# zhukovanadezhda/collaborative-filtering

Hardware: AMD Instinct MI355X
Metric: ratings/sec per ALS iteration at k=64 (higher is better)
Workload: dtype f32 (storage, solve, accumulate); Gram products as 2-way fp16 split (error <= 2^-23) on fp16 MFMA; rows over the condition limit redone in f64 (solve_dtype=auto)

## Files before the change

### collaborative-filtering_amd/csrc/row_solve.hip

```cpp
#include <type_traits>
#include "als_device.hpp"
#include "als_hip.h"
#include "row_common.hpp"
#include "slot_fold.hpp"

namespace {

template <int KB>
struct RowAcc {
    f32x4 acc[KCfg<KB>::NACC];
    float rhs[KB];
    float cs[KB];
    float sumr;
    float sumr2;
    __device__ __forceinline__ void zero() {
#pragma unroll
        for (int a = 0; a < KCfg<KB>::NACC; ++a) acc[a] = f32x4{0.f, 0.f, 0.f, 0.f};
#pragma unroll
        for (int b = 0; b < KB; ++b) { rhs[b] = 0.f; cs[b] = 0.f; }
        sumr = 0.f; sumr2 = 0.f;
    }
};

template <int KB, bool FULL>
__device__ __forceinline__ void process_chunk(RowAcc<KB>& A, int off_l, float r_l, int nvalid,
                                              const float* __restrict__ Fc, int q) {
    constexpr int GS = KCfg<KB>::GS;
#pragma unroll
    for (int g0 = 0; g0 < 16; g0 += GS) {
        if (!FULL && 4 * g0 >= nvalid) break;
        float f[GS][KB];
        int off_t[GS];
        float r_t[GS];
#pragma unroll
        for (int s = 0; s < GS; ++s) {
            const int src = FULL ? 16 * q + g0 + s : 4 * (g0 + s) + q;
            off_t[s] = bperm_i(off_l, src);
            r_t[s] = bperm_f(r_l, src);
        }
#pragma unroll
        for (int s = 0; s < GS; ++s)
            if (FULL || 4 * (g0 + s) < nvalid) load_frow<KB>(Fc + (uint32_t)off_t[s], f[s]);
#pragma unroll
        for (int s = 0; s < GS; ++s) {
            if (FULL || 4 * (g0 + s) < nvalid) {
#pragma unroll
                for (int b = 0; b < KB; ++b) {
                    A.rhs[b] = fmaf(f[s][b], r_t[s], A.rhs[b]);
                    A.cs[b] += f[s][b];
                }
#pragma unroll
                for (int bi = 0; bi < KB; ++bi)
#pragma unroll
                    for (int bj = 0; bj <= bi; ++bj)
                        A.acc[blk_idx(bi, bj)] = __builtin_amdgcn_mfma_f32_16x16x4f32(
                            f[s][bi], f[s][bj], A.acc[blk_idx(bi, bj)], 0, 0, 0);
            }
        }
    }
}


template <int KB, bool FULL>
__device__ __forceinline__ void process_chunk_f16x2(RowAcc<KB>& A, int off_l, float r_l, int nvalid,
                                                    const float* __restrict__ Fc, int q, float S) {
#pragma unroll
    for (int g = 0; g < 2; ++g) {
        if (!FULL && 32 * g >= nvalid) break;
        int off_t[8];
        float r_t[8];
        float f[8][KB];
#pragma unroll
        for (int j = 0; j < 8; ++j) {
            const int src = FULL ? 16 * q + 8 * g + j : 32 * g + 8 * q + j;
            off_t[j] = bperm_i(off_l, src);
            r_t[j] = bperm_f(r_l, src);
        }
#pragma unroll
        for (int j = 0; j < 8; ++j) load_frow<KB>(Fc + (uint32_t)off_t[j], f[j]);
        i32x4 H[KB], L[KB];
#pragma unroll
        for (int b = 0; b < KB; ++b) {
#pragma unroll
            for (int j = 0; j < 8; j += 2) {
                const float x0 = f[j][b], x1 = f[j + 1][b];
                A.rhs[b] = fmaf(x0, r_t[j], A.rhs[b]);
                A.rhs[b] = fmaf(x1, r_t[j + 1], A.rhs[b]);
                A.cs[b] += x0 + x1;
                int hw, lw;
                split2(x0, x1, S, hw, lw);
                H[b][j >> 1] = hw; L[b][j >> 1] = lw;
            }
        }
#pragma unroll
        for (int bi = 0; bi < KB; ++bi)
#pragma unroll
            for (int bj = 0; bj <= bi; ++bj) {
                f32x4 acc = A.acc[blk_idx(bi, bj)];
                const h16x8 hi = __builtin_bit_cast(h16x8, H[bi]), hj = __builtin_bit_cast(h16x8, H[bj]);
                const h16x8 li = __builtin_bit_cast(h16x8, L[bi]), lj = __builtin_bit_cast(h16x8, L[bj]);
                acc = __builtin_amdgcn_mfma_f32_16x16x32_f16(li, hj, acc, 0, 0, 0);
                acc = __builtin_amdgcn_mfma_f32_16x16x32_f16(hi, lj, acc, 0, 0, 0);
                acc = __builtin_amdgcn_mfma_f32_16x16x32_f16(hi, hj, acc, 0, 0, 0);
                A.acc[blk_idx(bi, bj)] = acc;
            }
    }
}

template <int KB, bool FULL>
__device__ __forceinline__ void process_chunk_planes(RowAcc<KB>& A, f32x4 (&E)[KB], int off_l, int rp_l, int nvalid,
                                                     const uint32_t* __restrict__ Pc, int q, int sel_c, int ones_c) {
    static_assert(KB == 4 || KB == 8, "pre-split operands: k = 49 ... 64 and 113 ... 128");
    constexpr int NW = KB / 2;
    typedef uint32_t u32x4 __attribute__((ext_vector_type(4)));
#pragma unroll
    for (int g = 0; g < 2; ++g) {
        if (!FULL && 32 * g >= nvalid) break;
        int off_t[8], rp_t[8];
#pragma unroll
        for (int j = 0; j < 8; ++j) {
            const int src = FULL ? 16 * q + 8 * g + j : 32 * g + 8 * q + j;
            off_t[j] = bperm_i(off_l, src);
            rp_t[j] = bperm_i(rp_l, src);
        }
        uint32_t w[8][KB];
#pragma unroll
        for (int j = 0; j < 8; ++j)
#pragma unroll
            for (int v4 = 0; v4 < KB / 4; ++v4) {
                const u32x4 t = *reinterpret_cast<const u32x4*>(Pc + (uint32_t)off_t[j] + 4 * v4);
                w[j][4 * v4] = t[0]; w[j][4 * v4 + 1] = t[1]; w[j][4 * v4 + 2] = t[2]; w[j][4 * v4 + 3] = t[3];
            }
        i32x4 H[KB], L[KB], R;
#pragma unroll
        for (int d = 0; d < 4; ++d) {
            R[d] = (int)__builtin_amdgcn_perm((uint32_t)rp_t[2 * d + 1], (uint32_t)rp_t[2 * d], (uint32_t)sel_c) | ones_c;
#pragma unroll
            for (int b = 0; b < KB; ++b) {
                const uint32_t sel = (b & 1) ? 0x07060302u : 0x05040100u;
                H[b][d] = (int)__builtin_amdgcn_perm(w[2 * d + 1][b >> 1], w[2 * d][b >> 1], sel);
                L[b][d] = (int)__builtin_amdgcn_perm(w[2 * d + 1][NW + (b >> 1)], w[2 * d][NW + (b >> 1)], sel);
            }
        }
        const h16x8 rr = __builtin_bit_cast(h16x8, R);
#pragma unroll
        for (int bi = 0; bi < KB; ++bi) {
            const h16x8 hi = __builtin_bit_cast(h16x8, H[bi]), li = __builtin_bit_cast(h16x8, L[bi]);
            E[bi] = __builtin_amdgcn_mfma_f32_16x16x32_f16(rr, li, E[bi], 0, 0, 0);
            E[bi] = __builtin_amdgcn_mfma_f32_16x16x32_f16(rr, hi, E[bi], 0, 0, 0);
#pragma unroll
            for (int bj = 0; bj <= bi; ++bj) {
                f32x4 acc = A.acc[blk_idx(bi, bj)];
                const h16x8 hj = __builtin_bit_cast(h16x8, H[bj]), lj = __builtin_bit_cast(h16x8, L[bj]);
                acc = __builtin_amdgcn_mfma_f32_16x16x32_f16(li, hj, acc, 0, 0, 0);
                acc = __builtin_amdgcn_mfma_f32_16x16x32_f16(hi, lj, acc, 0, 0, 0);
                acc = __builtin_amdgcn_mfma_f32_16x16x32_f16(hi, hj, acc, 0, 0, 0);
                A.acc[blk_idx(bi, bj)] = acc;
            }
        }
    }
}

template <int KB>
__device__ __forceinline__ void fold_planes_rhs(RowAcc<KB>& A, f32x4 (&E)[KB], int q, float inv_s) {
#pragma unroll
    for (int b = 0; b < KB; ++b) {
        A.rhs[b] += (q == 0) ? (E[b][0] + E[b][2]) * inv_s : 0.f;
        A.cs[b] += (q == 0) ? E[b][1] * inv_s : 0.f;
        E[b] = f32x4{0.f, 0.f, 0.f, 0.f};
    }
}

constexpr int FLUSH_GROUPS = 16;

template <int KB>
__device__ __forceinline__ void flush_acc(RowAcc<KB>& A, float* __restrict__ Ls, int lane, bool first) {
    if (!first) {
#pragma unroll
        for (int a = 0; a < KCfg<KB>::NACC; ++a)
#pragma unroll
            for (int r = 0; r < 4; ++r) A.acc[a][r] += Ls[(a * 4 + r) * 64 + lane];
    }
#pragma unroll
    for (int a = 0; a < KCfg<KB>::NACC; ++a)
#pragma unroll
        for (int r = 0; r < 4; ++r) {
            Ls[(a * 4 + r) * 64 + lane] = A.acc[a][r];
            A.acc[a][r] = 0.f;
        }
}

template <int KB>
__device__ __forceinline__ void unflush_acc(RowAcc<KB>& A, const float* __restrict__ Ls, int lane) {
#pragma unroll
    for (int a = 0; a < KCfg<KB>::NACC; ++a)
#pragma unroll
        for (int r = 0; r < 4; ++r) A.acc[a][r] += Ls[(a * 4 + r) * 64 + lane];
}

template <int KB, int MODE>
__device__ __forceinline__ void gram_accumulate(RowAcc<KB>& A, const int32_t* __restrict__ idxp,
                                                const float* __restrict__ valp, int len,
                                                const float* __restrict__ F, int ld, int zero_row,
                                                const float* __restrict__ bias_other, float mu,
                                                float bself, int lane, float* __restrict__ Ls, float S,
                                                const uint32_t* __restrict__ planes = nullptr) {
    const int c = lane & 15, q = lane >> 4;
    const float* Fc = F + KB * c;
    int nflush = 0;
    f32x4 E[MODE == 2 ? KB : 1];
    const uint32_t* Pc = planes + KB * c;
    const int sel_c = (c == 0) ? 0x05040100 : (c == 2) ? 0x07060302 : 0x0c0c0c0c;
    const int ones_c = (c == 1) ? 0x3C003C00 : 0;
    const float inv_s = __int_as_float((254 - ((__float_as_int(S) >> 23) & 0xff)) << 23);
    if constexpr (MODE == 2) {
#pragma unroll
        for (int b = 0; b < KB; ++b) E[b] = f32x4{0.f, 0.f, 0.f, 0.f};
    }
    int idx1 = (lane < len) ? __builtin_nontemporal_load(idxp + lane) : zero_row;
    int idx2 = (64 + lane < len) ? __builtin_nontemporal_load(idxp + 64 + lane) : zero_row;
    float val1 = (lane < len) ? __builtin_nontemporal_load(valp + lane) : 0.f;
    float bo1 = (lane < len) ? bias_other[idx1] : 0.f;
    for (int base = 0; base < len; base += 64) {
        const int idx0 = idx1;
        const float val0 = val1, bo0 = bo1;
        idx1 = idx2;
        const int t2 = base + 128 + lane;
        idx2 = (t2 < len) ? __builtin_nontemporal_load(idxp + t2) : zero_row;
        const int t1 = base + 64 + lane;
        val1 = (t1 < len) ? __builtin_nontemporal_load(valp + t1) : 0.f;
        bo1 = (t1 < len) ? bias_other[idx1] : 0.f;
        const int nvalid = min(64, len - base);
        const bool ok = lane < nvalid;
        const float rb = val0 - mu - bo0;
        A.sumr += ok ? rb : 0.f;
        A.sumr2 = ok ? fmaf(rb, rb, A.sumr2) : A.sumr2;
        const float r0 = ok ? (rb - bself) : 0.f;
        const int off0 = idx0 * ld;
        if constexpr (MODE == 0) {
            if (nvalid == 64) process_chunk<KB, true>(A, off0, r0, 64, Fc, q);
            else              process_chunk<KB, false>(A, off0, r0, nvalid, Fc, q);
        } else {
            if constexpr (MODE == 2) {
                const _Float16 rh = (_Float16)r0;
                const _Float16 rl = (_Float16)(r0 - (float)rh);
                const int rp = (int)__builtin_bit_cast(unsigned short, rh) | ((int)__builtin_bit_cast(unsigned short, rl) << 16);
                if (nvalid == 64) process_chunk_planes<KB, true>(A, E, off0, rp, 64, Pc, q, sel_c, ones_c);
                else              process_chunk_planes<KB, false>(A, E, off0, rp, nvalid, Pc, q, sel_c, ones_c);
            } else {
                if (nvalid == 64) process_chunk_f16x2<KB, true>(A, off0, r0, 64, Fc, q, S);
                else              process_chunk_f16x2<KB, false>(A, off0, r0, nvalid, Fc, q, S);
            }
            if (((base >> 6) + 1) % (FLUSH_GROUPS / 2) == 0 && base + 64 < len) {
                mfma_results_settle();
                if constexpr (MODE == 2) fold_planes_rhs<KB>(A, E, q, inv_s);
                flush_acc<KB>(A, Ls, lane, nflush == 0);
                ++nflush;
            }
        }
    }
    if (MODE != 0) mfma_results_settle();
    if constexpr (MODE == 2) fold_planes_rhs<KB>(A, E, q, inv_s);
    if (MODE != 0 && nflush > 0) {
        unflush_acc<KB>(A, Ls, lane);
        wave_lds_sync();
    }
}

template <int KB>
__device__ __forceinline__ void store_partial(const RowAcc<KB>& A, float* __restrict__ ws, int lane) {
    int it = 0;
#pragma unroll
    for (int a = 0; a < KCfg<KB>::NACC; ++a)
#pragma unroll
        for (int r = 0; r < 4; ++r) ws[(it++) * 64 + lane] = A.acc[a][r];
#pragma unroll
    for (int b = 0; b < KB; ++b) ws[(it++) * 64 + lane] = A.rhs[b];
#pragma unroll
    for (int b = 0; b < KB; ++b) ws[(it++) * 64 + lane] = A.cs[b];
    ws[(it++) * 64 + lane] = A.sumr;
    ws[it * 64 + lane] = A.sumr2;
}

template <int KB>
__device__ __forceinline__ void add_partial(RowAcc<KB>& A, const float* __restrict__ ws, int lane) {
    int it = 0;
#pragma unroll
    for (int a = 0; a < KCfg<KB>::NACC; ++a)
#pragma unroll
        for (int r = 0; r < 4; ++r) A.acc[a][r] += ws[(it++) * 64 + lane];
#pragma unroll
    for (int b = 0; b < KB; ++b) A.rhs[b] += ws[(it++) * 64 + lane];
#pragma unroll
    for (int b = 0; b < KB; ++b) A.cs[b] += ws[(it++) * 64 + lane];
    A.sumr += ws[(it++) * 64 + lane];
    A.sumr2 += ws[it * 64 + lane];
}

template <int KB, int J, int T, bool SOLVE>
__device__ __forceinline__ void panel_pivot(float (&p)[KCfg<KB>::NR][16], Chol<KB>& S, int lane) {
    constexpr int NR = KCfg<KB>::NR;
    constexpr int PIV = 16 * J + T, RP = PIV >> 6, LP = PIV & 63;
    constexpr int DR = (16 * J) >> 6, DL = (16 * J) & 63;
    const float prep = bperm_f(p[DR][T], DL + (lane & 15));
    const float d = readlane_f(p[RP][T], LP);
    const float inv = __builtin_amdgcn_rsqf(d);
    float l[NR];
#pragma unroll
    for (int rr = 0; rr < NR; ++rr) { l[rr] = p[rr][T] * inv; p[rr][T] = l[rr]; }
    float lrep = -(prep * inv);
    asm("s_nop 1" : "+v"(lrep));
    float yt = 0.f;
    if constexpr (SOLVE) yt = readlane_f(S.b[RP], LP) * inv;
    panel_trailing<KB, T + 1>(p, l, lrep);
    if constexpr (SOLVE) {
#pragma unroll
        for (int rr = 0; rr < NR; ++rr) S.b[rr] = fmaf(-l[rr], yt, S.b[rr]);
        S.y[RP] = select_lanes<1ull << LP>(yt, S.y[RP]);
    }
}

template <int KB, int J, int T, bool SOLVE>
__device__ __forceinline__ void panel_pivots(float (&p)[KCfg<KB>::NR][16], Chol<KB>& S, int lane) {
    if constexpr (T < 16) {
        panel_pivot<KB, J, T, SOLVE>(p, S, lane);
        panel_pivots<KB, J, T + 1, SOLVE>(p, S, lane);
    }
}

template <int KB, int J, bool SOLVE>
__device__ __forceinline__ void chol_panel(RowAcc<KB>& A, Chol<KB>& S, float* __restrict__ Ls, int lane) {
    using C = KCfg<KB>;
    constexpr int KP = C::KP, NR = C::NR;
    constexpr int OFF = C::lcol_off(J);
    const int c = lane & 15, q = lane >> 4;
    {
        const int swzc = (((c >> 2) ^ q) << 2) + (c & 3);
#pragma unroll
        for (int I = J; I < KB; ++I)
#pragma unroll
            for (int r = 0; r < 4; ++r)
                Ls[OFF + (16 * (I - J) + 4 * q + r) * 16 + swzc] = A.acc[blk_idx(I, J)][r];
    }
    wave_lds_sync();
    float p[NR][16];
    const int si = (lane >> 2) & 3;
#pragma unroll
    for (int rr = 0; rr < NR; ++rr) {
        const int i = lane + 64 * rr;
        const int rowi = min(max(i, 16 * J), KP - 1) - 16 * J;
#pragma unroll
        for (int g = 0; g < 4; ++g) {
            const f32x4 v = *reinterpret_cast<const f32x4*>(Ls + OFF + rowi * 16 + ((g ^ si) << 2));
            p[rr][4 * g] = v.x; p[rr][4 * g + 1] = v.y; p[rr][4 * g + 2] = v.z; p[rr][4 * g + 3] = v.w;
        }
    }
    wave_lds_sync();
    panel_pivots<KB, J, 0, SOLVE>(p, S, lane);
#pragma unroll
    for (int rr = 0; rr < NR; ++rr) {
        const int i = lane + 64 * rr;
        if (i >= 16 * J && i < KP) {
#pragma unroll
            for (int g = 0; g < 4; ++g) {
                const f32x4 v = {p[rr][4 * g], p[rr][4 * g + 1], p[rr][4 * g + 2], p[rr][4 * g + 3]};
                *reinterpret_cast<f32x4*>(Ls + OFF + (i - 16 * J) * 16 + ((g ^ si) << 2)) = v;
            }
        }
    }
    wave_lds_sync();
    {
        constexpr int DR = (16 * J) >> 6, DL = (16 * J) & 63;
        const float dl = Ls[OFF + c * 16 + (c & 3)];
        S.di[DR] = select_lanes<0xFFFFull << DL>(__builtin_amdgcn_rcpf(dl), S.di[DR]);
    }
    if constexpr (J + 1 < KB) {
        f32x4 op[KB - J - 1];
        const int sg = ((q ^ ((c >> 2) & 3)) << 2);
#pragma unroll
        for (int I = J + 1; I < KB; ++I)
            op[I - J - 1] = *reinterpret_cast<const f32x4*>(Ls + OFF + (16 * (I - J) + c) * 16 + sg);
#pragma unroll
        for (int K = J + 1; K < KB; ++K) {
            const f32x4 nb = -op[K - J - 1];
#pragma unroll
            for (int I = K; I < KB; ++I)
#pragma unroll
                for (int e = 0; e < 4; ++e)
                    A.acc[blk_idx(I, K)] = __builtin_amdgcn_mfma_f32_16x16x4f32(
                        op[I - J - 1][e], nb[e], A.acc[blk_idx(I, K)], 0, 0, 0);
        }
    }
}

template <int KB, int J, bool SOLVE>
__device__ __forceinline__ void chol_panels(RowAcc<KB>& A, Chol<KB>& S, float* __restrict__ Ls, int lane) {
    if constexpr (J < KB) {
        chol_panel<KB, J, SOLVE>(A, S, Ls, lane);
        chol_panels<KB, J + 1, SOLVE>(A, S, Ls, lane);
    }
}

template <int KB>
__device__ __forceinline__ bool row_needs_f64(const Chol<KB>& S, const als_row_solve_params& P, int row, bool spd,
                                              float mean_eig, float short_row_bound, int lane) {
    float dmx = 0.f, dmn = 0.f;
#pragma unroll
    for (int rr = 0; rr < KCfg<KB>::NR; ++rr) {
        const bool in = lane + 64 * rr < KCfg<KB>::KP;
        const float d = in ? S.di[rr] : 0.f;
        dmx = fmaxf(dmx, d);
        dmn = fmaxf(dmn, in ? __builtin_amdgcn_rcpf(d) : 0.f);
    }
    dmx = wave_max_nonneg(fmaxf(dmx, 0.f));
    dmn = wave_max_nonneg(fmaxf(dmn, 0.f));
    const float r = dmx * dmn;
    const float kappa = spd ? fmaxf(fmaxf(r * r, mean_eig * dmx * dmx), short_row_bound) : __builtin_inff();
    if (P.cond_out && lane == 0) P.cond_out[row] = kappa;
    const bool redo = !(kappa <= P.cond_limit);
    if (redo && lane == 0) P.redo_rows[atomicAdd(P.redo_count, 1)] = row;
    return redo;
}

template <int KB>
__device__ __forceinline__ float gram_trace(const RowAcc<KB>& A, int lane) {
    const int c = lane & 15, q = lane >> 4;
    float t = 0.f;
#pragma unroll
    for (int J = 0; J < KB; ++J) {
        const f32x4 a = A.acc[blk_idx(J, J)];
        const float lo = (c & 1) ? a[1] : a[0], hi = (c & 1) ? a[3] : a[2];
        t += (c & 2) ? hi : lo;
    }
    return wave_sum((q == (c >> 2)) ? t : 0.f);
}

template <int KB>
__device__ __forceinline__ void finish_row(RowAcc<KB>& A, const als_row_solve_params& P, int row,
                                           float* __restrict__ Ls, int lane) {
    using C = KCfg<KB>;
    constexpr int KP = C::KP, NR = C::NR;
    const int c = lane & 15, q = lane >> 4;
    const int64_t r64 = row;

    if (P.gram_mode == ALS_GRAM_F16X2) {
        const float un = P.F_scale[1];
#pragma unroll
        for (int a = 0; a < C::NACC; ++a) A.acc[a] *= un;
    }

#pragma unroll
    for (int b = 0; b < KB; ++b) {
        A.rhs[b] += __shfl_xor(A.rhs[b], 16, 64); A.rhs[b] += __shfl_xor(A.rhs[b], 32, 64);
        A.cs[b] += __shfl_xor(A.cs[b], 16, 64);   A.cs[b] += __shfl_xor(A.cs[b], 32, 64);
    }
    const float sumr = wave_sum(A.sumr);
    const float sumr2 = wave_sum(A.sumr2);

    Chol<KB> S;
    float csrow[NR];
    int colrow[NR];
#pragma unroll
    for (int rr = 0; rr < NR; ++rr) {
        float bsel = 0.f, csel = 0.f;
#pragma unroll
        for (int e = 0; e < 4; ++e) {
            constexpr int dummy = 0; (void)dummy;
            const int b = (4 * rr + e < KB) ? 4 * rr + e : KB - 1;
            if (4 * rr + e < KB) {
                bsel = (q == e) ? A.rhs[b] : bsel;
                csel = (q == e) ? A.cs[b] : csel;
            }
        }
        S.b[rr] = bsel; S.di[rr] = 0.f; S.y[rr] = 0.f;
        csrow[rr] = csel;
        colrow[rr] = perm_to_col<KB>(min(lane + 64 * rr, KP - 1));
    }

    if (P.gram_out) {
        float* G = P.gram_out + r64 * KP * KP;
#pragma unroll
        for (int I = 0; I < KB; ++I)
#pragma unroll
            for (int K = 0; K <= I; ++K)
#pragma unroll
                for (int r = 0; r < 4; ++r)
                    G[(16 * I + 4 * q + r) * KP + 16 * K + c] = A.acc[blk_idx(I, K)][r];
    }
#pragma unroll
    for (int rr = 0; rr < NR; ++rr) {
        const int i = lane + 64 * rr;
        if (i < KP) {
            if (P.rhs_out) P.rhs_out[r64 * KP + i] = S.b[rr];
            if (P.colsum_out) P.colsum_out[r64 * KP + i] = csrow[rr];
        }
    }
    if (P.sumr_out && lane == 0) P.sumr_out[row] = sumr;
    if (P.sumr2_out && lane == 0) P.sumr2_out[row] = sumr2;

    const float lam = (P.lambda_row ? P.lambda_row[row] : P.lambda_scalar) + ALS_EPS
                    + (P.diag_extra ? P.diag_extra[row] : 0.f);
    float mean_eig = 0.f, short_row_bound = 0.f;
    if (P.cond_limit > 0.f) {
        const int64_t nrat = P.indptr[row + 1] - P.indptr[row];
        mean_eig = gram_trace<KB>(A, lane) / fmaxf((float)min((int64_t)P.k, nrat), 1.f) + lam;
        short_row_bound = (nrat < 4 * (int64_t)P.k) ? mean_eig / lam : 0.f;
    }
#pragma unroll
    for (int J = 0; J < KB; ++J) {
        const float dv = (perm_to_col<KB>(16 * J + c) < P.k) ? lam : 1.0f;
#pragma unroll
        for (int r = 0; r < 4; ++r) A.acc[blk_idx(J, J)][r] += (4 * q + r == c) ? dv : 0.f;
    }

    if (P.factor_out) {
        chol_panels<KB, 0, false>(A, S, Ls, lane);
        const bool spd = chol_spd<KB>(S, lane);
        if (P.cond_limit > 0.f) {
            if (row_needs_f64<KB>(S, P, row, spd, mean_eig, short_row_bound, lane)) return;
        } else if (!spd && lane == 0) atomicMax(P.status, row + 1);
        float* M = P.factor_out + r64 * KP * KP;
#pragma unroll
        for (int rr = 0; rr < NR; ++rr) {
            const int i = lane + 64 * rr;
            const int ic = min(i, KP - 1);
            const int colb = C::lcol_off_rt(ic >> 4) - 16 * (ic >> 4) * 16 + (c & 3);
#pragma unroll 8
            for (int p = 0; p < KP; ++p) {
                const int Jp = p >> 4;
                const int rowv = max(ic, 16 * Jp);
                const float lrow = Ls[C::lcol_off_rt(Jp) + (rowv - 16 * Jp) * 16 +
                                      ((((p >> 2) & 3) ^ ((rowv >> 2) & 3)) << 2) + (p & 3)];
                const int rsafe = max(p, ic & ~15);
                const float lcolv = Ls[colb + rsafe * 16 + (((c >> 2) ^ ((rsafe >> 2) & 3)) << 2)];
                if (i < KP) __builtin_nontemporal_store((p == i) ? S.di[rr] : (p < i ? lrow : lcolv), M + p * KP + i);
            }
        }
        return;
    }

    float rhs0[NR];
#pragma unroll
    for (int rr = 0; rr < NR; ++rr) rhs0[rr] = S.b[rr];
    if (P.rhs_extra) {
#pragma unroll
        for (int rr = 0; rr < NR; ++rr)
            if (lane + 64 * rr < KP) S.b[rr] += P.rhs_extra[r64 * P.ld + colrow[rr]];
    }
    if (!(P.reserved0 & 2)) {
        chol_panels<KB, 0, true>(A, S, Ls, lane);
        const bool spd = chol_spd<KB>(S, lane);
        if (P.cond_limit > 0.f) {
            if (row_needs_f64<KB>(S, P, row, spd, mean_eig, short_row_bound, lane)) return;
        } else if (!spd && lane == 0) atomicMax(P.status, row + 1);
    }
    float x[NR];
    if (!(P.reserved0 & 4)) backward_solve<KB>(Ls, S, x, lane);
    else {
#pragma unroll
        for (int rr = 0; rr < NR; ++rr) x[rr] = S.y[rr];
    }

    float dot = 0.f, xr = 0.f, yy = 0.f, xx = 0.f;
#pragma unroll
    for (int rr = 0; rr < NR; ++rr) {
        if (lane + 64 * rr < KP) {
            dot = fmaf(csrow[rr], x[rr], dot);
            xr = fmaf(rhs0[rr], x[rr], xr);
            yy = fmaf(S.y[rr], S.y[rr], yy);
            xx = fmaf(x[rr], x[rr], xx);
        }
    }
    dot = wave_sum(dot);
    const float nnz = (float)(P.indptr[row + 1] - P.indptr[row]);
    const float lb = P.lambda_bias_row ? P.lambda_bias_row[row] : P.lambda_bias_scalar;
    const float bnew = (sumr - dot) / (nnz + lb + ALS_EPS);
    const float bold = P.bias_self[row];
    float st1 = 0.f, st2 = 0.f;
    if (P.stat_out) {
        xr = wave_sum(xr); yy = wave_sum(yy); xx = wave_sum(xx);
        const double bn = bnew, dt = dot;
        const double s1 = (double)sumr - (double)nnz * bn;
        const double s2 = (double)sumr2 - 2.0 * bn * (double)sumr + (double)nnz * bn * bn;
        const double cross = (double)xr + ((double)bold - bn) * dt;
        const double quad = (double)yy - (double)lam * (double)xx;
        const double sd2 = s2 - 2.0 * cross + quad;
        if (P.cond_limit > 0.f && !(sd2 >= 1e-3 * s2)) {
            if (lane == 0) P.redo_rows[atomicAdd(P.redo_count, 1)] = row;
            return;
        }
        st1 = (float)(s1 - dt);
        st2 = (float)sd2;
    }
#pragma unroll
    for (int rr = 0; rr < NR; ++rr)
        if (lane + 64 * rr < KP) P.X_out[r64 * P.ld + colrow[rr]] = x[rr];
    __builtin_amdgcn_sched_barrier(0);
    if (lane == 0) {
        P.bias_out[row] = bnew;
        if (P.stat_out) { P.stat_out[2 * r64] = st1; P.stat_out[2 * r64 + 1] = st2; }
    }
}

template <int KB, int MODE>
__global__ __launch_bounds__(64 * KCfg<KB>::WPW, KCfg<KB>::MINW)
void k_row_tasks(const als_row_solve_params P) {
    using C = KCfg<KB>;
    __shared__ __attribute__((aligned(16))) float lds_all[C::WPW * C::LDS_FLOATS];
    const int lane = threadIdx.x & 63;
    const int wave = threadIdx.x >> 6;
    const int wave_u = wave;
    const int64_t tid = (int64_t)blockIdx.x * C::WPW + wave_u;
    if (tid >= P.ntasks) return;
    const als_task t = P.tasks[tid];
    const int row = t.row;
    const int seg = t.seg;
    const int slot = t.slot;
    const int64_t rbeg = P.indptr[row], rend = P.indptr[row + 1];
    const int64_t beg = rbeg + (int64_t)seg * ALS_SPLIT_CHUNK;
    const int len = (int)min((int64_t)ALS_SPLIT_CHUNK, rend - beg);
    const float mu = (float)(*P.mu);
    const float bself = P.bias_self[row];

    const float S = (MODE != 0) ? P.F_scale[0] : 1.f;

    RowAcc<KB> A;
    A.zero();
    if (!(P.reserved0 & 1))
        gram_accumulate<KB, MODE>(A, P.indices + beg, P.vals + beg, len, P.F, P.ld, P.F_zero_row,
                                  P.bias_other, mu, bself, lane, lds_all + wave * C::LDS_FLOATS, S,
                                  (const uint32_t*)P.F_planes);
    if (slot >= 0) {
        store_partial<KB>(A, (float*)P.workspace + (size_t)slot * C::SLOT_ITEMS * 64, lane);
        return;
    }
    finish_row<KB>(A, P, row, lds_all + wave_u * C::LDS_FLOATS, lane);
}

template <int KB, int NB>
__device__ __forceinline__ void row_dual(const als_row_solve_params& P, int row, int64_t beg, int len,
                                         float* __restrict__ Ls, int lane) {
    constexpr int KP = KCfg<KB>::KP, NR = KCfg<KB>::NR, NSLAB = (KP + 31) / 32;
    constexpr int NS = KCfg<NB>::NR;
    const int c = lane & 15, q = lane >> 4;
    const float bold = P.bias_self[row];
    const float mu = (float)*P.mu;
    bool ok[NS];
    int idx_l[NS];
    float r_l[NS];
#pragma unroll
    for (int ss = 0; ss < NS; ++ss) {
        const int t = lane + 64 * ss;
        ok[ss] = t < len;
        idx_l[ss] = ok[ss] ? P.indices[beg + t] : P.F_zero_row;
        r_l[ss] = ok[ss] ? (P.vals[beg + t] - mu - P.bias_other[idx_l[ss]]) - bold : 0.f;
    }
    const int nblk = (len + 15) >> 4;
    int off[NB];
#pragma unroll
    for (int I = 0; I < NB; ++I)
        off[I] = bperm_i(idx_l[(16 * I) >> 6], (16 * I + c) & 63) * P.ld;

    const float Sc = P.F_scale[0];
    RowAcc<NB> A;
    A.zero();
    for (int s = 0; s < NSLAB; ++s) {
        const bool in = 32 * s + 8 * q < KP;
        i32x4 H[NB], L[NB];
#pragma unroll
        for (int I = 0; I < NB; ++I) {
            float f[8];
            if (I < nblk && in) {
                const f32x4 v0 = *reinterpret_cast<const f32x4*>(P.F + (uint32_t)off[I] + 32 * s + 8 * q);
                const f32x4 v1 = *reinterpret_cast<const f32x4*>(P.F + (uint32_t)off[I] + 32 * s + 8 * q + 4);
                f[0] = v0.x; f[1] = v0.y; f[2] = v0.z; f[3] = v0.w; f[4] = v1.x; f[5] = v1.y; f[6] = v1.z; f[7] = v1.w;
            } else {
#pragma unroll
                for (int e = 0; e < 8; ++e) f[e] = 0.f;
            }
#pragma unroll
            for (int e = 0; e < 8; e += 2) {
                int hw, lw;
                split2(f[e], f[e + 1], Sc, hw, lw);
                H[I][e >> 1] = hw; L[I][e >> 1] = lw;
            }
        }
#pragma unroll
        for (int bi = 0; bi < NB; ++bi)
#pragma unroll
            for (int bj = 0; bj <= bi; ++bj) {
                if (bi >= nblk) continue;
                f32x4 acc = A.acc[blk_idx(bi, bj)];
                const h16x8 hi = __builtin_bit_cast(h16x8, H[bi]), hj = __builtin_bit_cast(h16x8, H[bj]);
                const h16x8 li = __builtin_bit_cast(h16x8, L[bi]), lj = __builtin_bit_cast(h16x8, L[bj]);
                acc = __builtin_amdgcn_mfma_f32_16x16x32_f16(li, hj, acc, 0, 0, 0);
                acc = __builtin_amdgcn_mfma_f32_16x16x32_f16(hi, lj, acc, 0, 0, 0);
                acc = __builtin_amdgcn_mfma_f32_16x16x32_f16(hi, hj, acc, 0, 0, 0);
                A.acc[blk_idx(bi, bj)] = acc;
            }
    }
    mfma_results_settle();
    {
        const float un = P.F_scale[1];
#pragma unroll
        for (int a = 0; a < KCfg<NB>::NACC; ++a) A.acc[a] *= un;
    }
    const float lam = (P.lambda_row ? P.lambda_row[row] : P.lambda_scalar) + ALS_EPS;
    const float dual_mean_eig = (P.cond_limit > 0.f) ? gram_trace<NB>(A, lane) / (float)max(min(len, P.k), 1) + lam : 0.f;
#pragma unroll
    for (int J = 0; J < NB; ++J) {
        const float dv = (16 * J + c < len) ? lam : 1.0f;
#pragma unroll
        for (int r = 0; r < 4; ++r) A.acc[blk_idx(J, J)][r] += (4 * q + r == c) ? dv : 0.f;
    }
    Chol<NB> S;
#pragma unroll
    for (int ss = 0; ss < NS; ++ss) { S.b[ss] = r_l[ss]; S.di[ss] = 0.f; S.y[ss] = 0.f; }
    chol_panels<NB, 0, true>(A, S, Ls, lane);
    {
        const bool spd = chol_spd<NB>(S, lane);
        if (P.cond_limit > 0.f) {
            if (row_needs_f64<NB>(S, P, row, spd, dual_mean_eig, dual_mean_eig / lam, lane)) return;
        } else if (!spd && lane == 0) atomicMax(P.status, row + 1);
    }
    float w[NS];
    backward_solve<NB>(Ls, S, w, lane);

    float x[NR];
#pragma unroll
    for (int rr = 0; rr < NR; ++rr) x[rr] = 0.f;
#pragma unroll
    for (int ss = 0; ss < NS; ++ss) {
        const int lim = min(len - 64 * ss, 64);
        for (int i0 = 0; i0 < lim; i0 += 8) {
            float fv[8][NR], wi[8];
#pragma unroll
            for (int u = 0; u < 8; ++u) {
                const int i = min(i0 + u, 63);
                wi[u] = (i0 + u < lim) ? readlane_f(w[ss], i) : 0.f;
                const int o = __builtin_amdgcn_readlane(idx_l[ss], i) * P.ld;
#pragma unroll
                for (int rr = 0; rr < NR; ++rr) fv[u][rr] = P.F[(uint32_t)o + min(lane + 64 * rr, KP - 1)];
            }
#pragma unroll
            for (int u = 0; u < 8; ++u)
#pragma unroll
                for (int rr = 0; rr < NR; ++rr) x[rr] = fmaf(fv[u][rr], wi[u], x[rr]);
        }
    }
    const int64_t r64 = row;
#pragma unroll
    for (int rr = 0; rr < NR; ++rr)
        if (lane + 64 * rr < KP) P.X_out[r64 * P.ld + lane + 64 * rr] = x[rr];
    const float nnz = (float)len;
    const float lb = P.lambda_bias_row ? P.lambda_bias_row[row] : P.lambda_bias_scalar;
    float wsum = 0.f;
#pragma unroll
    for (int ss = 0; ss < NS; ++ss) wsum += ok[ss] ? w[ss] : 0.f;
    const float sw = wave_sum(wsum);
    const float bnew = (nnz * bold + lam * sw) / (nnz + lb + ALS_EPS);
    if (lane == 0) P.bias_out[row] = bnew;
    if (P.stat_out) {
        float e1 = 0.f, e2 = 0.f;
#pragma unroll
        for (int ss = 0; ss < NS; ++ss) {
            const float e = ok[ss] ? (bold - bnew) + lam * w[ss] : 0.f;
            e1 += e;
            e2 = fmaf(e, e, e2);
        }
        const float s1 = wave_sum(e1), s2 = wave_sum(e2);
        if (lane == 0) { P.stat_out[2 * r64] = s1; P.stat_out[2 * r64 + 1] = s2; }
    }
}

template <int KB>
__global__ __launch_bounds__(256, 3)
void k_row_dual(const als_row_solve_params P, int64_t task0, int64_t ntail) {
    using C4 = KCfg<4>;
    __shared__ __attribute__((aligned(16))) float lds_all[4 * C4::LDS_FLOATS];
    const int lane = threadIdx.x & 63, wave = threadIdx.x >> 6;
    const int64_t tid = (int64_t)blockIdx.x * 4 + wave;
    if (tid >= ntail) return;
    float* Ls = lds_all + wave * C4::LDS_FLOATS;
    const int row = P.tasks[task0 + tid].row;
    const int64_t beg = P.indptr[row];
    const int len = (int)(P.indptr[row + 1] - beg);
    if (len > 64 || len < 1) {
        if (lane == 0) atomicMax(P.status, row + 1);
        return;
    }
    if (len <= 16) row_dual<KB, 1>(P, row, beg, len, Ls, lane);
    else if (len <= 32) row_dual<KB, 2>(P, row, beg, len, Ls, lane);
    else if (len <= 48) row_dual<KB, 3>(P, row, beg, len, Ls, lane);
    else row_dual<KB, 4>(P, row, beg, len, Ls, lane);
}

template <int KB>
__global__ __launch_bounds__(128, 2)
void k_row_dual_mid(const als_row_solve_params P, int64_t task0, int64_t nmid) {
    using C6 = KCfg<6>;
    __shared__ __attribute__((aligned(16))) float lds_all[2 * C6::LDS_FLOATS];
    const int lane = threadIdx.x & 63, wave = threadIdx.x >> 6;
    const int64_t tid = (int64_t)blockIdx.x * 2 + wave;
    if (tid >= nmid) return;
    float* Ls = lds_all + wave * C6::LDS_FLOATS;
    const int row = P.tasks[task0 + tid].row;
    const int64_t beg = P.indptr[row];
    const int len = (int)(P.indptr[row + 1] - beg);
    if (len > 96 || len <= 64) {
        if (lane == 0) atomicMax(P.status, row + 1);
        return;
    }
    if (len <= 80) row_dual<KB, 5>(P, row, beg, len, Ls, lane);
    else row_dual<KB, 6>(P, row, beg, len, Ls, lane);
}

template <int KB>
__global__ __launch_bounds__(64 * KCfg<KB>::WPW, KCfg<KB>::MINW)
void k_row_long(const als_row_solve_params P) {
    using C = KCfg<KB>;
    __shared__ __attribute__((aligned(16))) float lds_all[C::WPW * C::LDS_FLOATS];
    const int lane = threadIdx.x & 63;
    const int wave = threadIdx.x >> 6;
    const int64_t tid = (int64_t)blockIdx.x * C::WPW + wave;
    if (tid >= P.nlong) return;
    const als_long_row lr = P.long_rows[tid];
    RowAcc<KB> A;
    A.zero();
    add_partial<KB>(A, (const float*)P.workspace + (size_t)lr.slot0 * C::SLOT_ITEMS * 64, lane);
    finish_row<KB>(A, P, lr.row, lds_all + wave * C::LDS_FLOATS, lane);
}

template <int KB>
struct SumSlots {
    static constexpr int NV = KCfg<KB>::SLOT_ITEMS * 16;
    static constexpr int GROUPS = (NV + 63) / 64;
};

template <int KB>
__global__ __launch_bounds__(64)
void k_sum_slots(const als_long_row* __restrict__ long_rows, float* __restrict__ workspace) {
    constexpr int NV = SumSlots<KB>::NV, G = SumSlots<KB>::GROUPS;
    const als_long_row lr = long_rows[blockIdx.x / G];
    const int e = (blockIdx.x % G) * 64 + threadIdx.x;
    if (e >= NV || lr.nslots < 2) return;
    f32x4* w0 = reinterpret_cast<f32x4*>(workspace) + (size_t)lr.slot0 * NV + e;
    w0[0] = slot_fold::fold<true>(w0, (size_t)NV, lr.nslots);
}

__global__ __launch_bounds__(256)
void k_factor_scale(const float* __restrict__ F, int64_t n4, float* __restrict__ scale, int32_t* __restrict__ redo_count) {
    __shared__ uint32_t wmax[4];
    const f32x4* __restrict__ F4 = reinterpret_cast<const f32x4*>(F);
    uint32_t m = 0;
    const int64_t stride = (int64_t)gridDim.x * 256;
    for (int64_t i = (int64_t)blockIdx.x * 256 + threadIdx.x; i < n4; i += 4 * stride) {
        f32x4 v[4];
#pragma unroll
        for (int u = 0; u < 4; ++u)
            v[u] = (i + u * stride < n4) ? F4[i + u * stride] : f32x4{0.f, 0.f, 0.f, 0.f};
#pragma unroll
        for (int u = 0; u < 4; ++u)
#pragma unroll
            for (int e = 0; e < 4; ++e) m = max(m, (uint32_t)__float_as_int(v[u][e]) & 0x7FFFFFFFu);
    }
#pragma unroll
    for (int o = 32; o >= 1; o >>= 1) m = max(m, (uint32_t)__shfl_xor((int)m, o, 64));
    if ((threadIdx.x & 63) == 0) wmax[threadIdx.x >> 6] = m;
    __syncthreads();
    if (threadIdx.x == 0) {
        uint32_t* w = reinterpret_cast<uint32_t*>(scale);
        atomicMax(&w[2], max(max(wmax[0], wmax[1]), max(wmax[2], wmax[3])));
        __threadfence();
        if (atomicAdd(&w[3], 1u) == gridDim.x - 1) {
            __threadfence();
            const uint32_t mx = atomicMax(&w[2], 0u);
            const int e = (int)(mx >> 23);
            const int se = min(max(268 - e, 67), 187);
            scale[0] = __int_as_float(se << 23);
            scale[1] = __int_as_float((381 - 2 * se) << 23);
            atomicExch(&w[2], 0u);
            atomicExch(&w[3], 0u);
            if (redo_count) *redo_count = 0;
        }
    }
}

int launch_factor_scale(const float* F, int64_t nfloats, float* scale, int32_t* redo_count, hipStream_t st) {
    const int64_t n4 = nfloats / 4;
    const unsigned grid = (unsigned)min((int64_t)512, max((int64_t)1, (n4 + 1023) / 1024));
    hipLaunchKernelGGL(k_factor_scale, dim3(grid), dim3(256), 0, st, F, n4, scale, redo_count);
    return hipGetLastError() == hipSuccess ? 0 : ALS_E_LAUNCH;
}

__global__ void k_reset_word(int32_t* w) { *w = 0; }

template <int KB>
__global__ __launch_bounds__(256)
void k_split_planes(const float* __restrict__ F, int64_t npieces, const float* __restrict__ scale,
                    uint32_t* __restrict__ planes) {
    typedef uint32_t u32x4 __attribute__((ext_vector_type(4)));
    const float S = scale[0];
    for (int64_t e = (int64_t)blockIdx.x * 256 + threadIdx.x; e < npieces; e += (int64_t)gridDim.x * 256) {
        uint32_t h[KB / 2], l[KB / 2];
#pragma unroll
        for (int v4 = 0; v4 < KB / 4; ++v4) {
            const f32x4 x = reinterpret_cast<const f32x4*>(F)[e * (KB / 4) + v4];
            int h01, l01, h23, l23;
            split2(x[0], x[1], S, h01, l01);
            split2(x[2], x[3], S, h23, l23);
            h[2 * v4] = (uint32_t)h01; h[2 * v4 + 1] = (uint32_t)h23;
            l[2 * v4] = (uint32_t)l01; l[2 * v4 + 1] = (uint32_t)l23;
        }
        if constexpr (KB == 4) {
            reinterpret_cast<u32x4*>(planes)[e] = u32x4{h[0], h[1], l[0], l[1]};
        } else {
            reinterpret_cast<u32x4*>(planes)[2 * e] = u32x4{h[0], h[1], h[2], h[3]};
            reinterpret_cast<u32x4*>(planes)[2 * e + 1] = u32x4{l[0], l[1], l[2], l[3]};
        }
    }
}

template <int KB>
int launch_row_solve(const als_row_solve_params* p, hipStream_t st) {
    using C = KCfg<KB>;
    const bool plain = p->gram_mode == ALS_GRAM_F16X2 && p->reserved0 == 0 && p->X_out && p->bias_out &&
                       !p->gram_out && !p->factor_out && !p->rhs_out && !p->colsum_out && !p->sumr_out &&
                       !p->sumr2_out && !p->rhs_extra && !p->diag_extra;
    int64_t ntail = 0, nmid = 0;
    if (plain && p->ndual_tail >= 0 && p->ndual_mid >= 0 && (int64_t)p->ndual_tail + p->ndual_mid <= p->ntasks) {
        ntail = p->ndual_tail;
        if constexpr (KB >= 7) nmid = p->ndual_mid;
    }
    const int64_t nprimal = p->ntasks - ntail - nmid;
    if (nprimal > 0) {
        als_row_solve_params q = *p;
        q.ntasks = nprimal;
        const unsigned grid = (unsigned)((nprimal + C::WPW - 1) / C::WPW);
        bool planes = false;
        if constexpr (KB == 4 || KB == 8)
            planes = p->gram_mode == ALS_GRAM_F16X2 && p->F_planes != nullptr && p->reserved0 == 0;
        if (planes) {
            if constexpr (KB == 4 || KB == 8) {
                const int64_t npieces = ((int64_t)p->F_zero_row + 1) * 16;
                const unsigned sgrid = (unsigned)min((int64_t)4096, (npieces + 255) / 256);
                hipLaunchKernelGGL(k_split_planes<KB>, dim3(sgrid), dim3(256), 0, st, p->F, npieces, p->F_scale,
                                   (uint32_t*)p->F_planes);
                hipLaunchKernelGGL((k_row_tasks<KB, 2>), dim3(grid), dim3(64 * C::WPW), 0, st, q);
            }
        } else if (p->gram_mode == ALS_GRAM_F16X2)
            hipLaunchKernelGGL((k_row_tasks<KB, 1>), dim3(grid), dim3(64 * C::WPW), 0, st, q);
        else
            hipLaunchKernelGGL((k_row_tasks<KB, 0>), dim3(grid), dim3(64 * C::WPW), 0, st, q);
    }
    {
        if (ntail > 0)
            hipLaunchKernelGGL(k_row_dual<KB>, dim3((unsigned)((ntail + 3) / 4)), dim3(256), 0, st, *p, nprimal + nmid, ntail);
    }
    if constexpr (KB >= 7) {
        if (nmid > 0)
            hipLaunchKernelGGL(k_row_dual_mid<KB>, dim3((unsigned)((nmid + 1) / 2)), dim3(128), 0, st, *p, nprimal, nmid);
    }
    if (p->nlong > 0) {
        if (p->nlong * SumSlots<KB>::GROUPS > (int64_t)0x7FFFFFFF) return ALS_E_BADARG;
        hipLaunchKernelGGL(k_sum_slots<KB>, dim3((unsigned)(p->nlong * SumSlots<KB>::GROUPS)), dim3(64), 0, st,
                           p->long_rows, (float*)p->workspace);
        const unsigned grid = (unsigned)((p->nlong + C::WPW - 1) / C::WPW);
        hipLaunchKernelGGL(k_row_long<KB>, dim3(grid), dim3(64 * C::WPW), 0, st, *p);
    }
    return hipGetLastError() == hipSuccess ? 0 : ALS_E_LAUNCH;
}

}

int als_row_solve_f64_dispatch(const als_row_solve_params* p, hipStream_t st);
int als_row_redo_f64_dispatch(const als_row_solve_params* p, hipStream_t st);

extern "C" int als_version(void) { return ALS_HIP_VERSION; }
extern "C" int als_padded_k(int k) { return (k < 1 || k > ALS_MAX_K) ? ALS_E_BADK : 16 * ((k + 15) / 16); }
extern "C" int als_perm_index(int k, int c) {
    const int ld = als_padded_k(k);
    if (ld < 0 || c < 0 || c >= ld) return ALS_E_BADARG;
    const int KB = ld / 16;
    return 16 * (c % KB) + c / KB;
}
extern "C" int64_t als_partial_slot_bytes(int k) {
    const int ld = als_padded_k(k);
    if (ld < 0) return ALS_E_BADK;
    const int KB = ld / 16;
    return (int64_t)(KB * (KB + 1) / 2 * 4 + 2 * KB + 2) * 64 * sizeof(float);
}

extern "C" int als_factor_scale(const float* F, int64_t nfloats, float* scale, void* stream) {
    if (!F || !scale || nfloats < 0 || (nfloats & 3) || ((uintptr_t)F & 15)) return ALS_E_BADARG;
    return launch_factor_scale(F, nfloats, scale, nullptr, (hipStream_t)stream);
}

extern "C" int als_row_solve(const als_row_solve_params* p, void* stream) {
    if (!p) return ALS_E_BADARG;
    const int ld = als_padded_k(p->k);
    if (ld < 0) return ALS_E_BADK;
    if (p->ld != ld || !p->indptr || !p->indices || !p->vals || !p->F || !p->bias_self ||
        !p->bias_other || !p->mu || !p->status || p->ntasks < 0 || p->nlong < 0 || p->F_zero_row < 0 ||
        (p->gram_mode != ALS_GRAM_F32 && p->gram_mode != ALS_GRAM_F16X2 && p->gram_mode != ALS_GRAM_F64) ||
        (int64_t)p->F_zero_row * ld >= ((int64_t)1 << 31))
        return ALS_E_BADARG;
    if (p->ntasks > 0 && !p->tasks) return ALS_E_BADARG;
    if (p->nlong > 0 && (!p->long_rows || !p->workspace)) return ALS_E_BADARG;
    if (p->factor_out) {
        if (!p->rhs_out || !p->colsum_out || !p->sumr_out) return ALS_E_BADARG;
    } else if (!p->X_out || !p->bias_out) {
        return ALS_E_BADARG;
    }
    hipStream_t st = (hipStream_t)stream;
    if (p->gram_mode == ALS_GRAM_F64) return als_row_solve_f64_dispatch(p, st);
    const bool redo = p->cond_limit > 0.f;
    if (redo && (!p->redo_count || !p->redo_rows)) return ALS_E_BADARG;
    bool counter_reset = false;
    if (p->gram_mode == ALS_GRAM_F16X2) {
        if (!p->F_scale) return ALS_E_BADARG;
        if (!p->F_scale_ready) {
            const int rc = launch_factor_scale(p->F, ((int64_t)p->F_zero_row + 1) * ld, p->F_scale,
                                               redo ? p->redo_count : nullptr, st);
            if (rc != 0) return rc;
            counter_reset = true;
        }
    }
    if (redo && !counter_reset) hipLaunchKernelGGL(k_reset_word, dim3(1), dim3(1), 0, st, p->redo_count);
    int rc = ALS_E_BADK;
#ifdef ALS_KB_ONLY
    if (ld / 16 == ALS_KB_ONLY) rc = launch_row_solve<ALS_KB_ONLY>(p, st);
#else
    ALS_DISPATCH_KB(ld / 16, rc = launch_row_solve<KB>(p, st));
#endif
    if (rc == 0 && redo) rc = als_row_redo_f64_dispatch(p, st);
    return rc;
}
```

Baseline: 8.945 billion.

## Peel first Gram chunk, fold unscale into solve, reload task after accumulation

The first 64-rating chunk is peeled so accumulators start from the first MFMA result instead of being zeroed and then accumulated into. In f16x2 mode the finish step no longer multiplies every Gram accumulator by the unscale factor; instead lambda, the identity padding and the RHS are scaled by a power of two, which is valid when no Gram or factor outputs are requested. The task record is also reloaded after accumulation, with readfirstlane and asm barriers, to shorten live ranges and cut register pressure across the Gram loop. For the k=64 f16x2 path, peeling and reload are gated by a macro that defaults to off, so only the scaled-solve change clearly applies there. These changes add template complexity and small numeric differences from the scaling.

```diff
diff --git a/collaborative-filtering_amd/csrc/row_solve.hip b/collaborative-filtering_amd/csrc/row_solve.hip
--- a/collaborative-filtering_amd/csrc/row_solve.hip
+++ b/collaborative-filtering_amd/csrc/row_solve.hip
@@ -22,13 +22,13 @@
     }
 };
 
-template <int KB, bool FULL>
+template <int KB, bool FULL, bool FIRST>
 __device__ __forceinline__ void process_chunk(RowAcc<KB>& A, int off_l, float r_l, int nvalid,
                                               const float* __restrict__ Fc, int q) {
     constexpr int GS = KCfg<KB>::GS;
 #pragma unroll
     for (int g0 = 0; g0 < 16; g0 += GS) {
-        if (!FULL && 4 * g0 >= nvalid) break;
+        if (!FULL && !(FIRST && g0 == 0) && 4 * g0 >= nvalid) break;
         float f[GS][KB];
         int off_t[GS];
         float r_t[GS];
@@ -40,33 +40,35 @@
         }
 #pragma unroll
         for (int s = 0; s < GS; ++s)
-            if (FULL || 4 * (g0 + s) < nvalid) load_frow<KB>(Fc + (uint32_t)off_t[s], f[s]);
+            if (FULL || (FIRST && g0 + s == 0) || 4 * (g0 + s) < nvalid) load_frow<KB>(Fc + (uint32_t)off_t[s], f[s]);
 #pragma unroll
         for (int s = 0; s < GS; ++s) {
-            if (FULL || 4 * (g0 + s) < nvalid) {
+            const bool start = FIRST && g0 + s == 0;
+            if (FULL || start || 4 * (g0 + s) < nvalid) {
 #pragma unroll
                 for (int b = 0; b < KB; ++b) {
-                    A.rhs[b] = fmaf(f[s][b], r_t[s], A.rhs[b]);
-                    A.cs[b] += f[s][b];
+                    A.rhs[b] = fmaf(f[s][b], r_t[s], start ? 0.f : A.rhs[b]);
+                    A.cs[b] = (start ? 0.f : A.cs[b]) + f[s][b];
                 }
 #pragma unroll
                 for (int bi = 0; bi < KB; ++bi)
 #pragma unroll
                     for (int bj = 0; bj <= bi; ++bj)
                         A.acc[blk_idx(bi, bj)] = __builtin_amdgcn_mfma_f32_16x16x4f32(
-                            f[s][bi], f[s][bj], A.acc[blk_idx(bi, bj)], 0, 0, 0);
-            }
-        }
-    }
-}
-
-
-template <int KB, bool FULL>
+                            f[s][bi], f[s][bj], start ? f32x4{0.f, 0.f, 0.f, 0.f} : A.acc[blk_idx(bi, bj)], 0, 0, 0);
+            }
+        }
+    }
+}
+
+
+template <int KB, bool FULL, bool FIRST>
 __device__ __forceinline__ void process_chunk_f16x2(RowAcc<KB>& A, int off_l, float r_l, int nvalid,
                                                     const float* __restrict__ Fc, int q, float S) {
 #pragma unroll
     for (int g = 0; g < 2; ++g) {
-        if (!FULL && 32 * g >= nvalid) break;
+        const bool start = FIRST && g == 0;
+        if (!FULL && !start && 32 * g >= nvalid) break;
         int off_t[8];
         float r_t[8];
         float f[8][KB];
@@ -84,9 +86,9 @@
 #pragma unroll
             for (int j = 0; j < 8; j += 2) {
                 const float x0 = f[j][b], x1 = f[j + 1][b];
-                A.rhs[b] = fmaf(x0, r_t[j], A.rhs[b]);
+                A.rhs[b] = fmaf(x0, r_t[j], (start && j == 0) ? 0.f : A.rhs[b]);
                 A.rhs[b] = fmaf(x1, r_t[j + 1], A.rhs[b]);
-                A.cs[b] += x0 + x1;
+                A.cs[b] = ((start && j == 0) ? 0.f : A.cs[b]) + (x0 + x1);
                 int hw, lw;
                 split2(x0, x1, S, hw, lw);
                 H[b][j >> 1] = hw; L[b][j >> 1] = lw;
@@ -96,7 +98,7 @@
         for (int bi = 0; bi < KB; ++bi)
 #pragma unroll
             for (int bj = 0; bj <= bi; ++bj) {
-                f32x4 acc = A.acc[blk_idx(bi, bj)];
+                f32x4 acc = start ? f32x4{0.f, 0.f, 0.f, 0.f} : A.acc[blk_idx(bi, bj)];
                 const h16x8 hi = __builtin_bit_cast(h16x8, H[bi]), hj = __builtin_bit_cast(h16x8, H[bj]);
                 const h16x8 li = __builtin_bit_cast(h16x8, L[bi]), lj = __builtin_bit_cast(h16x8, L[bj]);
                 acc = __builtin_amdgcn_mfma_f32_16x16x32_f16(li, hj, acc, 0, 0, 0);
@@ -107,7 +109,7 @@
     }
 }
 
-template <int KB, bool FULL>
+template <int KB, bool FULL, bool FIRST>
 __device__ __forceinline__ void process_chunk_planes(RowAcc<KB>& A, f32x4 (&E)[KB], int off_l, int rp_l, int nvalid,
                                                      const uint32_t* __restrict__ Pc, int q, int sel_c, int ones_c) {
     static_assert(KB == 4 || KB == 8, "pre-split operands: k = 49 ... 64 and 113 ... 128");
@@ -115,7 +117,8 @@
     typedef uint32_t u32x4 __attribute__((ext_vector_type(4)));
 #pragma unroll
     for (int g = 0; g < 2; ++g) {
-        if (!FULL && 32 * g >= nvalid) break;
+        const bool start = FIRST && g == 0;
+        if (!FULL && !start && 32 * g >= nvalid) break;
         int off_t[8], rp_t[8];
 #pragma unroll
         for (int j = 0; j < 8; ++j) {
@@ -146,11 +149,11 @@
 #pragma unroll
         for (int bi = 0; bi < KB; ++bi) {
             const h16x8 hi = __builtin_bit_cast(h16x8, H[bi]), li = __builtin_bit_cast(h16x8, L[bi]);
-            E[bi] = __builtin_amdgcn_mfma_f32_16x16x32_f16(rr, li, E[bi], 0, 0, 0);
+            E[bi] = __builtin_amdgcn_mfma_f32_16x16x32_f16(rr, li, start ? f32x4{0.f, 0.f, 0.f, 0.f} : E[bi], 0, 0, 0);
             E[bi] = __builtin_amdgcn_mfma_f32_16x16x32_f16(rr, hi, E[bi], 0, 0, 0);
 #pragma unroll
             for (int bj = 0; bj <= bi; ++bj) {
-                f32x4 acc = A.acc[blk_idx(bi, bj)];
+                f32x4 acc = start ? f32x4{0.f, 0.f, 0.f, 0.f} : A.acc[blk_idx(bi, bj)];
                 const h16x8 hj = __builtin_bit_cast(h16x8, H[bj]), lj = __builtin_bit_cast(h16x8, L[bj]);
                 acc = __builtin_amdgcn_mfma_f32_16x16x32_f16(li, hj, acc, 0, 0, 0);
                 acc = __builtin_amdgcn_mfma_f32_16x16x32_f16(hi, lj, acc, 0, 0, 0);
@@ -161,17 +164,34 @@
     }
 }
 
-template <int KB>
+template <int KB, bool START, bool RESTART>
 __device__ __forceinline__ void fold_planes_rhs(RowAcc<KB>& A, f32x4 (&E)[KB], int q, float inv_s) {
 #pragma unroll
     for (int b = 0; b < KB; ++b) {
-        A.rhs[b] += (q == 0) ? (E[b][0] + E[b][2]) * inv_s : 0.f;
-        A.cs[b] += (q == 0) ? E[b][1] * inv_s : 0.f;
-        E[b] = f32x4{0.f, 0.f, 0.f, 0.f};
+        if constexpr (START) {
+            A.rhs[b] = (q == 0) ? fmaf(E[b][0] + E[b][2], inv_s, 0.f) : 0.f;
+            A.cs[b] = (q == 0) ? fmaf(E[b][1], inv_s, 0.f) : 0.f;
+        } else {
+            A.rhs[b] += (q == 0) ? (E[b][0] + E[b][2]) * inv_s : 0.f;
+            A.cs[b] += (q == 0) ? E[b][1] * inv_s : 0.f;
+        }
+        if (RESTART) E[b] = f32x4{0.f, 0.f, 0.f, 0.f};
     }
 }
 
 constexpr int FLUSH_GROUPS = 16;
+
+#ifndef ALS_FW_VSTEP64
+#define ALS_FW_VSTEP64 0
+#endif
+template <int KB, int MODE>
+struct FixedWork {
+    static constexpr bool V64 = KB == 4 && MODE == 1;
+    static constexpr bool PEEL = V64 ? (ALS_FW_VSTEP64 & 1) != 0 : (KB <= 9 || MODE != 0);
+    static constexpr bool RELOAD = V64 ? (ALS_FW_VSTEP64 & 2) != 0 : KB <= 5;
+};
+template <int KB>
+constexpr bool SCALED_SOLVE = KB <= 8;
 
 template <int KB>
 __device__ __forceinline__ void flush_acc(RowAcc<KB>& A, float* __restrict__ Ls, int lane, bool first) {
@@ -213,15 +233,13 @@
     const int sel_c = (c == 0) ? 0x05040100 : (c == 2) ? 0x07060302 : 0x0c0c0c0c;
     const int ones_c = (c == 1) ? 0x3C003C00 : 0;
     const float inv_s = __int_as_float((254 - ((__float_as_int(S) >> 23) & 0xff)) << 23);
-    if constexpr (MODE == 2) {
-#pragma unroll
-        for (int b = 0; b < KB; ++b) E[b] = f32x4{0.f, 0.f, 0.f, 0.f};
-    }
     int idx1 = (lane < len) ? __builtin_nontemporal_load(idxp + lane) : zero_row;
     int idx2 = (64 + lane < len) ? __builtin_nontemporal_load(idxp + 64 + lane) : zero_row;
     float val1 = (lane < len) ? __builtin_nontemporal_load(valp + lane) : 0.f;
     float bo1 = (lane < len) ? bias_other[idx1] : 0.f;
-    for (int base = 0; base < len; base += 64) {
+    constexpr bool PEEL = FixedWork<KB, MODE>::PEEL;
+    auto chunk = [&](auto first_c, int base) __attribute__((always_inline)) {
+        constexpr bool FIRST = decltype(first_c)::value;
         const int idx0 = idx1;
         const float val0 = val1, bo0 = bo1;
         idx1 = idx2;
@@ -233,34 +251,48 @@
         const int nvalid = min(64, len - base);
         const bool ok = lane < nvalid;
         const float rb = val0 - mu - bo0;
-        A.sumr += ok ? rb : 0.f;
-        A.sumr2 = ok ? fmaf(rb, rb, A.sumr2) : A.sumr2;
+        A.sumr = (FIRST ? 0.f : A.sumr) + (ok ? rb : 0.f);
+        A.sumr2 = FIRST ? (ok ? rb * rb : 0.f) : (ok ? fmaf(rb, rb, A.sumr2) : A.sumr2);
         const float r0 = ok ? (rb - bself) : 0.f;
         const int off0 = idx0 * ld;
         if constexpr (MODE == 0) {
-            if (nvalid == 64) process_chunk<KB, true>(A, off0, r0, 64, Fc, q);
-            else              process_chunk<KB, false>(A, off0, r0, nvalid, Fc, q);
+            if (nvalid == 64) process_chunk<KB, true, FIRST>(A, off0, r0, 64, Fc, q);
+            else              process_chunk<KB, false, FIRST>(A, off0, r0, nvalid, Fc, q);
         } else {
             if constexpr (MODE == 2) {
                 const _Float16 rh = (_Float16)r0;
                 const _Float16 rl = (_Float16)(r0 - (float)rh);
                 const int rp = (int)__builtin_bit_cast(unsigned short, rh) | ((int)__builtin_bit_cast(unsigned short, rl) << 16);
-                if (nvalid == 64) process_chunk_planes<KB, true>(A, E, off0, rp, 64, Pc, q, sel_c, ones_c);
-                else              process_chunk_planes<KB, false>(A, E, off0, rp, nvalid, Pc, q, sel_c, ones_c);
+                if (nvalid == 64) process_chunk_planes<KB, true, FIRST>(A, E, off0, rp, 64, Pc, q, sel_c, ones_c);
+                else              process_chunk_planes<KB, false, FIRST>(A, E, off0, rp, nvalid, Pc, q, sel_c, ones_c);
             } else {
-                if (nvalid == 64) process_chunk_f16x2<KB, true>(A, off0, r0, 64, Fc, q, S);
-                else              process_chunk_f16x2<KB, false>(A, off0, r0, nvalid, Fc, q, S);
-            }
-            if (((base >> 6) + 1) % (FLUSH_GROUPS / 2) == 0 && base + 64 < len) {
+                if (nvalid == 64) process_chunk_f16x2<KB, true, FIRST>(A, off0, r0, 64, Fc, q, S);
+                else              process_chunk_f16x2<KB, false, FIRST>(A, off0, r0, nvalid, Fc, q, S);
+            }
+            if (!FIRST && ((base >> 6) + 1) % (FLUSH_GROUPS / 2) == 0 && base + 64 < len) {
                 mfma_results_settle();
-                if constexpr (MODE == 2) fold_planes_rhs<KB>(A, E, q, inv_s);
+                if constexpr (MODE == 2) {
+                    if (PEEL && nflush == 0) fold_planes_rhs<KB, true, true>(A, E, q, inv_s);
+                    else                  fold_planes_rhs<KB, false, true>(A, E, q, inv_s);
+                }
                 flush_acc<KB>(A, Ls, lane, nflush == 0);
                 ++nflush;
             }
         }
-    }
+    };
+    static_assert(FLUSH_GROUPS / 2 > 1, "the peeled first chunk never flushes");
+    if constexpr (PEEL) {
+        chunk(std::true_type{}, 0);
+    } else if constexpr (MODE == 2) {
+#pragma unroll
+        for (int b = 0; b < KB; ++b) E[b] = f32x4{0.f, 0.f, 0.f, 0.f};
+    }
+    for (int base = PEEL ? 64 : 0; base < len; base += 64) chunk(std::false_type{}, base);
     if (MODE != 0) mfma_results_settle();
-    if constexpr (MODE == 2) fold_planes_rhs<KB>(A, E, q, inv_s);
+    if constexpr (MODE == 2) {
+        if (PEEL && nflush == 0) fold_planes_rhs<KB, true, false>(A, E, q, inv_s);
+        else                     fold_planes_rhs<KB, false, false>(A, E, q, inv_s);
+    }
     if (MODE != 0 && nflush > 0) {
         unflush_acc<KB>(A, Ls, lane);
         wave_lds_sync();
@@ -443,10 +475,18 @@
     const int c = lane & 15, q = lane >> 4;
     const int64_t r64 = row;
 
+    float s2 = 1.f;
     if (P.gram_mode == ALS_GRAM_F16X2) {
         const float un = P.F_scale[1];
-#pragma unroll
-        for (int a = 0; a < C::NACC; ++a) A.acc[a] *= un;
+        const int eu = (__float_as_int(un) >> 23) & 0xff;
+        const bool scaled = SCALED_SOLVE<KB> && !P.gram_out && !P.factor_out && !P.rhs_out && !P.colsum_out && !P.stat_out && !P.rhs_extra &&
+                            eu >= 127 - 60 && eu <= 127 + 60;
+        if (scaled) {
+            s2 = __int_as_float((254 - eu) << 23);
+        } else {
+#pragma unroll
+            for (int a = 0; a < C::NACC; ++a) A.acc[a] *= un;
+        }
     }
 
 #pragma unroll
@@ -472,7 +512,7 @@
                 csel = (q == e) ? A.cs[b] : csel;
             }
         }
-        S.b[rr] = bsel; S.di[rr] = 0.f; S.y[rr] = 0.f;
+        S.b[rr] = bsel * s2; S.di[rr] = 0.f; S.y[rr] = 0.f;
         csrow[rr] = csel;
         colrow[rr] = perm_to_col<KB>(min(lane + 64 * rr, KP - 1));
     }
@@ -498,8 +538,9 @@
     if (P.sumr_out && lane == 0) P.sumr_out[row] = sumr;
     if (P.sumr2_out && lane == 0) P.sumr2_out[row] = sumr2;
 
-    const float lam = (P.lambda_row ? P.lambda_row[row] : P.lambda_scalar) + ALS_EPS
-                    + (P.diag_extra ? P.diag_extra[row] : 0.f);
+    const float lam1 = (P.lambda_row ? P.lambda_row[row] : P.lambda_scalar) + ALS_EPS
+                     + (P.diag_extra ? P.diag_extra[row] : 0.f);
+    const float lam = lam1 * s2;
     float mean_eig = 0.f, short_row_bound = 0.f;
     if (P.cond_limit > 0.f) {
         const int64_t nrat = P.indptr[row + 1] - P.indptr[row];
@@ -508,7 +549,7 @@
     }
 #pragma unroll
     for (int J = 0; J < KB; ++J) {
-        const float dv = (perm_to_col<KB>(16 * J + c) < P.k) ? lam : 1.0f;
+        const float dv = (perm_to_col<KB>(16 * J + c) < P.k) ? lam : s2;
 #pragma unroll
         for (int r = 0; r < 4; ++r) A.acc[blk_idx(J, J)][r] += (4 * q + r == c) ? dv : 0.f;
     }
@@ -609,32 +650,51 @@
     __shared__ __attribute__((aligned(16))) float lds_all[C::WPW * C::LDS_FLOATS];
     const int lane = threadIdx.x & 63;
     const int wave = threadIdx.x >> 6;
-    const int wave_u = wave;
-    const int64_t tid = (int64_t)blockIdx.x * C::WPW + wave_u;
+    const int64_t tid = (int64_t)blockIdx.x * C::WPW + wave;
     if (tid >= P.ntasks) return;
-    const als_task t = P.tasks[tid];
+    int len;
+    float bself;
+    int64_t beg;
+    {
+        const als_task t = P.tasks[tid];
+        const int64_t rbeg = P.indptr[t.row], rend = P.indptr[t.row + 1];
+        beg = rbeg + (int64_t)t.seg * ALS_SPLIT_CHUNK;
+        len = (int)min((int64_t)ALS_SPLIT_CHUNK, rend - beg);
+        bself = P.bias_self[t.row];
+    }
+    const float mu = (float)(*P.mu);
+
+    const float S = (MODE != 0) ? P.F_scale[0] : 1.f;
+
+    RowAcc<KB> A;
+    if constexpr (FixedWork<KB, MODE>::PEEL) {
+        gram_accumulate<KB, MODE>(A, P.indices + beg, P.vals + beg, (P.reserved0 & 1) ? 0 : max(len, 0), P.F, P.ld,
+                                  P.F_zero_row, P.bias_other, mu, bself, lane, lds_all + wave * C::LDS_FLOATS, S,
+                                  (const uint32_t*)P.F_planes);
+    } else {
+        A.zero();
+        if (!(P.reserved0 & 1))
+            gram_accumulate<KB, MODE>(A, P.indices + beg, P.vals + beg, len, P.F, P.ld, P.F_zero_row,
+                                      P.bias_other, mu, bself, lane, lds_all + wave * C::LDS_FLOATS, S,
+                                      (const uint32_t*)P.F_planes);
+    }
+    int wave_u = wave, lane_t = lane;
+    if constexpr (FixedWork<KB, MODE>::RELOAD) {
+        int zero;
+        asm volatile("s_mov_b32 %0, 0" : "=s"(zero));
+        wave_u = __builtin_amdgcn_readfirstlane(wave) + zero;
+        lane_t = threadIdx.x;
+        asm volatile("" : "+v"(lane_t));
+        lane_t &= 63;
+    }
+    const als_task t = P.tasks[(int64_t)blockIdx.x * C::WPW + wave_u];
     const int row = t.row;
-    const int seg = t.seg;
     const int slot = t.slot;
-    const int64_t rbeg = P.indptr[row], rend = P.indptr[row + 1];
-    const int64_t beg = rbeg + (int64_t)seg * ALS_SPLIT_CHUNK;
-    const int len = (int)min((int64_t)ALS_SPLIT_CHUNK, rend - beg);
-    const float mu = (float)(*P.mu);
-    const float bself = P.bias_self[row];
-
-    const float S = (MODE != 0) ? P.F_scale[0] : 1.f;
-
-    RowAcc<KB> A;
-    A.zero();
-    if (!(P.reserved0 & 1))
-        gram_accumulate<KB, MODE>(A, P.indices + beg, P.vals + beg, len, P.F, P.ld, P.F_zero_row,
-                                  P.bias_other, mu, bself, lane, lds_all + wave * C::LDS_FLOATS, S,
-                                  (const uint32_t*)P.F_planes);
     if (slot >= 0) {
-        store_partial<KB>(A, (float*)P.workspace + (size_t)slot * C::SLOT_ITEMS * 64, lane);
+        store_partial<KB>(A, (float*)P.workspace + (size_t)slot * C::SLOT_ITEMS * 64, lane_t);
         return;
     }
-    finish_row<KB>(A, P, row, lds_all + wave_u * C::LDS_FLOATS, lane);
+    finish_row<KB>(A, P, row, lds_all + wave_u * C::LDS_FLOATS, lane_t);
 }
 
 template <int KB, int NB>
```

Measured after the change: 8.938 billion. No clear change (-0.1%).
